# JohannesBuchner/massivedatans

Measured on AMD Instinct MI355X. Metric: likelihood evals/sec across N datasets per constrained draw, higher is better.
Workload: dtype f64

## Files before the change

### massivedatans_amd/csrc/mdns_chunk.hip

```cpp
#include "mdns_quad.h"
#include <cstdlib>

namespace mdns {

typedef JointMailbox ChunkMailbox;

template <int NST>
__global__ __launch_bounds__(256) void k_chunk_accept(
    const double *__restrict__ Y, int ld, int nx, int nxp, const double *__restrict__ xgrid,
    const double *__restrict__ params, int B, double scale,
    const int *__restrict__ rows, int *__restrict__ rows_dev, int M, int ntiles,
    const double *__restrict__ higher, int *__restrict__ flags, int stamp, JointTrail trail, JointHeader *__restrict__ header)
{
	extern __shared__ __attribute__((aligned(16))) double lds[];
	if (blockIdx.x == 0 && threadIdx.x == 0) header->status = 0;
	double2 *tpl = reinterpret_cast<double2 *>(lds);
	double *par = lds + (size_t) nxp * 4;
	unsigned long long *votes = reinterpret_cast<unsigned long long *>(par + 12);
	const int lane = threadIdx.x & 63, wave = threadIdx.x >> 6;
	const int q = lane & 3;
	const int bt = blockIdx.x / ntiles, tile = blockIdx.x - bt * ntiles;
	double pv = 0.0;
	if (threadIdx.x < 12) {
		const int b = bt * 4 + threadIdx.x / 3;
		pv = b < B ? params[(size_t) b * 3 + threadIdx.x % 3] : 0.0;
	}
	const int r = wave * 16 + (lane >> 2);
	const int k = tile * 64 + r;
	const bool live = k < M;
	const int kk = live ? k : M - 1;
	const int row = rows ? rows[kk] : kk;
	if (rows_dev && bt == 0 && live && q == 0) rows_dev[k] = row;
	double2 y[NST];
	const double thr = quad_load_row<NST>(Y, ld, row, live, q, higher, y);
	if (threadIdx.x < 12) par[threadIdx.x] = pv;
	__syncthreads();
	quad_templates(lds, par, xgrid, nx, nxp, bt * 4, B);
	__syncthreads();
	const double L = quad_sum<NST>(tpl, nxp / kCH, q, y) * scale;
	quad_vote(L, thr, bt * 4 + q < B, bt * 4 + q, true, bt * 4 + wave, ntiles, tile, r, votes, flags, stamp, trail);
}

__global__ __launch_bounds__(1024) void k_chunk_commit(
    const int *__restrict__ thr_rows, int M, int B, int ntiles, const int *__restrict__ flags, int stamp,
    JointTrail trail, JointArrays st, JointHeader *__restrict__ header, unsigned long long *__restrict__ fillbits,
    ChunkMailbox *__restrict__ box, unsigned long long seq)
{
	__shared__ int s_first, s_status;
	if (threadIdx.x == 0) s_status = 0;
	const int bstar = first_flagged<1024>(&s_first, flags, B, [=](int f) { return f == stamp; });
	const int lane = threadIdx.x & 63, wave = threadIdx.x >> 6;
	if (bstar < B) {
		for (int tile = wave; tile < ntiles; tile += 16) {
			const size_t at = (size_t) bstar * ntiles + tile;
			const unsigned long long word = trail.stamp_of[at] == trail.stamp ? trail.word[at] : 0ull;
			const int k = tile * 64 + lane;
			if (k < M && (word >> lane & 1ull)) {
				const int d = thr_rows ? thr_rows[k] : k;
				if (!shelf_append<16>(st, d, trail.L[at * 64 + lane], st.higher[d])) atomicOr(&s_status, 1);
			}
			if (lane == 0) { fillbits[tile] = word; mail_store(&box->bits[tile], word); }
		}
	}
	handover_release();
	__syncthreads();
	if (threadIdx.x != 0) return;
	const int accepted = bstar < B ? bstar : -1;
	header->accepted = accepted;
	header->status = s_status;
	mail_store(&box->accepted, accepted);
	mail_store(&box->status, s_status);
	mail_raise(&box->seq, seq);
}

typedef double double4_t __attribute__((ext_vector_type(4)));
typedef double double2_t __attribute__((ext_vector_type(2)));
__device__ __forceinline__ double4_t gg_join(double2_t a, double2_t b) { return double4_t{a[0], a[1], b[0], b[1]}; }

template <int SPEC, int CHUNK, int DEPTH, int PROBE>
__global__ __launch_bounds__(256) void k_gauss_mfma_filter(
    const double *__restrict__ YT, int nxp, int nx, const double *__restrict__ model_t, const double *__restrict__ msq, int B,
    double scale, const int *__restrict__ thr_rows, int M, int ntiles, int nbt, int ngroups,
    const double *__restrict__ higher, const double *__restrict__ ysq, int *__restrict__ flags, int *__restrict__ ambiguous,
    int stamp, int *__restrict__ lowest)
{
	constexpr int NB = SPEC / 16;
	constexpr int kRow2 = SPEC / 2;
	constexpr int kPieces = (CHUNK * kRow2 + 255) / 256;
	constexpr bool kWhole = (CHUNK * kRow2) % 256 == 0;
	constexpr int kRowsPerPass = 256 / kRow2;
	constexpr int kSteps = CHUNK / 4;
	__shared__ __attribute__((aligned(16))) double stage[DEPTH + 1][CHUNK * SPEC];
	const int lane = threadIdx.x & 63, wave = threadIdx.x >> 6;
	const int xcd = blockIdx.x & 7, local = blockIdx.x >> 3;
	const int tile = (local / ngroups) * 8 + xcd, grp = local - (local / ngroups) * ngroups;
	if (tile >= ntiles) return;
	const int bt = grp * 4 + wave;
	const bool working = bt < nbt;
	const int kq = lane >> 4, jq = lane & 15;
	const double *ap = model_t + (size_t) (working ? bt : 0) * nxp * 16 + lane;
	const int first = tile * SPEC;
	const int prow = threadIdx.x / kRow2, pcol = threadIdx.x % kRow2;
	const double2 *src = reinterpret_cast<const double2 *>(YT + ((size_t) (first >> 6) * nxp << 6) + (first & 63)) + (size_t) prow * 32 + pcol;
	double2 piece[DEPTH + 1][kPieces];
	double a[DEPTH + 1][kSteps];
	double4_t acc[NB];
#pragma unroll
	for (int t = 0; t < NB; t++) acc[t] = double4_t{0, 0, 0, 0};
	const int nchunks = (nxp + CHUNK - 1) / CHUNK;
	const int nk = nxp / 4;
#define FILTER_FETCH(SET, CHUNK_NO) { \
	const int cn_ = (CHUNK_NO) < nchunks ? (CHUNK_NO) : nchunks - 1; \
	_Pragma("unroll") for (int i = 0; i < kPieces; i++) { \
		const int row = kWhole || prow + i * kRowsPerPass < CHUNK ? prow + i * kRowsPerPass : CHUNK - 1; \
		const int ch = cn_ * CHUNK + row; \
		piece[SET][i] = src[(size_t) ((ch < nxp ? ch : nxp - 1) - prow) * 32]; \
	} \
	_Pragma("unroll") for (int i = 0; i < kSteps; i++) { \
		const int k = cn_ * kSteps + i; \
		a[SET][i] = ap[(size_t) (k < nk ? k : nk - 1) * 64]; \
	} }
#define FILTER_STAGE(SET, CHUNK_NO) { \
	const int cn_ = (CHUNK_NO) < nchunks ? (CHUNK_NO) : nchunks - 1; \
	_Pragma("unroll") for (int i = 0; i < kPieces; i++) { \
		const int row = prow + i * kRowsPerPass; \
		const bool inside = cn_ * CHUNK + row < nxp; \
		double2 v = piece[SET][i]; \
		v.x = inside ? v.x : 0.0; v.y = inside ? v.y : 0.0; \
		if (kWhole || row < CHUNK) reinterpret_cast<double2 *>(stage[SET])[i * 256 + threadIdx.x] = v; \
	} }
#define FILTER_BODY(R, R1, RF, CHUNK_NO) { \
	const int c_ = (CHUNK_NO); \
	if (PROBE != 2 && PROBE != 3) FILTER_FETCH(RF, c_ + DEPTH) \
	if (working && c_ < nchunks && PROBE != 1) { \
		const double *cur = stage[R]; \
		double b[2][NB]; \
		_Pragma("unroll") for (int t = 0; t < NB; t++) b[0][t] = cur[kq * SPEC + jq + 16 * t]; \
		_Pragma("unroll") for (int i = 0; i < kSteps; i++) { \
			if (i + 1 < kSteps) { \
				_Pragma("unroll") for (int t = 0; t < NB; t++) b[(i + 1) & 1][t] = cur[((i + 1) * 4 + kq) * SPEC + jq + 16 * t]; \
			} \
			 \
			_Pragma("unroll") for (int t = 0; t < NB; t++) \
				acc[t] = __builtin_amdgcn_mfma_f64_16x16x4f64(a[R][i], PROBE == 3 ? a[R][(i + t + 1) % kSteps] : b[i & 1][t], acc[t], 0, 0, 0); \
		} \
	} \
	if (PROBE != 2 && PROBE != 3) FILTER_STAGE(R1, c_ + 1) \
	__syncthreads(); }
	FILTER_FETCH(0, 0)
	if (DEPTH == 2) FILTER_FETCH(1, 1)
	FILTER_STAGE(0, 0)
	__syncthreads();
	if (DEPTH == 2) {
#pragma unroll 1
		for (int c = 0; c < nchunks; c += 3) {
			FILTER_BODY(0, 1, 2, c)
			FILTER_BODY(1, 2 % (DEPTH + 1), 0, c + 1)
			FILTER_BODY(2 % (DEPTH + 1), 0, 1, c + 2)
		}
	} else {
#pragma unroll 1
		for (int c = 0; c < nchunks; c += 2) {
			FILTER_BODY(0, 1, 1, c)
			FILTER_BODY(1, 0, 0, c + 1)
		}
	}
#undef FILTER_BODY
#undef FILTER_STAGE
#undef FILTER_FETCH
	if (!working) return;
	if (PROBE == 3) { double sum = 0.0; for (int t = 0; t < NB; t++) sum += acc[t][t]; if (sum == 12345.678) flags[0] = 1; return; }
	const double unit = fabs(scale) * (double) (nx + 8) * 0x1p-52;
	double mm[4];
#pragma unroll
	for (int v = 0; v < 4; v++) mm[v] = msq[bt * 16 + 4 * v + kq];
	bool hit[4] = {false, false, false, false}, maybe[4] = {false, false, false, false};
#pragma unroll
	for (int t = 0; t < NB; t++) {
		const int k = first + 16 * t + jq;
		const bool live = k < M;
		const int kk = live ? k : M - 1;
		const int d = thr_rows ? thr_rows[kk] : kk;
		const double thr = live ? higher[d] : __builtin_nan("");
		const double yy = ysq[d];
#pragma unroll
		for (int v = 0; v < 4; v++) {
			const double S = acc[t][v];
			const double Lf = scale * ((mm[v] - 2.0 * S) + yy);
			const double E4 = 4.0 * unit * ((mm[v] + 2.0 * fabs(S)) + yy);
			const bool valid = bt * 16 + 4 * v + kq < B;
			const bool h = valid && Lf > thr + E4;
			hit[v] = hit[v] || h;
			maybe[v] = maybe[v] || (valid && !h && Lf >= thr - E4);
		}
	}
	int best = 0x7fffffff;
#pragma unroll
	for (int v = 0; v < 4; v++) {
		const unsigned long long hm = __ballot(hit[v]), mb = __ballot(maybe[v]);
		if (lane == 0) {
#pragma unroll
			for (int g = 0; g < 4; g++) {
				const int cand = bt * 16 + 4 * v + g;
				if ((hm >> (16 * g)) & 0xffffull) { flags[cand] = 1; best = cand < best ? cand : best; }
				else if ((mb >> (16 * g)) & 0xffffull) ambiguous[cand] = stamp;
			}
		}
	}
	if (lane == 0 && best != 0x7fffffff) atomicMax(lowest, B - best);
}

template <int NC>
__global__ __launch_bounds__(256) void k_gauss_mfma_direct(
    const double *__restrict__ YT, int nxp, int nx, const double *__restrict__ model_t, const double *__restrict__ msq, int B,
    double scale, const int *__restrict__ thr_rows, int M, int nbt,
    const double *__restrict__ higher, const double *__restrict__ ysq, int *__restrict__ flags, int *__restrict__ ambiguous,
    int stamp, int *__restrict__ lowest, const double *__restrict__ zeros)
{
	const int lane = threadIdx.x & 63, wave = __builtin_amdgcn_readfirstlane((int) (threadIdx.x >> 6));
	const int i = lane & 15, q = lane >> 4;
	const int first = blockIdx.x * 16;
	const int ct0 = (blockIdx.y * 4 + wave) * NC;
	if (ct0 >= nbt) return;
	const int sp = first + i;
	const double *pa = YT + ((size_t) (sp >> 6) * nxp << 6) + (sp & 63);
	const double *pb[NC];
#pragma unroll
	for (int c = 0; c < NC; c++) pb[c] = model_t + (size_t) (ct0 + c < nbt ? ct0 + c : nbt - 1) * nxp * 16 + i;
	double4_t acc[NC];
#pragma unroll
	for (int c = 0; c < NC; c++) acc[c] = double4_t{0, 0, 0, 0};
	const int ng = (nxp + 15) >> 4;
	double a[2][4], b[2][NC][4];
#define GD_FETCH(SET, G) { \
	const int g_ = (G) < ng ? (G) : ng - 1; \
	_Pragma("unroll") for (int t = 0; t < 4; t++) { \
		const int ch = 16 * g_ + 4 * q + t; \
		const bool in = ch < nxp && (G) < ng; \
		a[SET][t] = *(in ? pa + ((size_t) ch << 6) : zeros + i); \
		const int cb = ch < nxp ? ch : nxp - 1; \
		_Pragma("unroll") for (int c = 0; c < NC; c++) b[SET][c][t] = pb[c][(size_t) cb << 4]; \
	} }
#define GD_BODY(SET) { \
	__builtin_amdgcn_sched_barrier(0); \
	_Pragma("unroll") for (int t = 0; t < 4; t++) \
		_Pragma("unroll") for (int c = 0; c < NC; c++) \
			acc[c] = __builtin_amdgcn_mfma_f64_16x16x4f64(a[SET][t], b[SET][c][t], acc[c], 0, 0, 0); \
	__builtin_amdgcn_sched_barrier(0); }
	GD_FETCH(0, 0)
#pragma unroll 1
	for (int g = 0; g < ng; g += 2) {
		GD_FETCH(1, g + 1)
		GD_BODY(0)
		GD_FETCH(0, g + 2)
		GD_BODY(1)
	}
#undef GD_BODY
#undef GD_FETCH
	const double unit = fabs(scale) * (double) (nx + 8) * 0x1p-52;
	double thr[4], yy[4];
#pragma unroll
	for (int v = 0; v < 4; v++) {
		const int k = first + 4 * v + q;
		const bool live = k < M;
		const int kk = live ? k : M - 1;
		const int d = thr_rows ? thr_rows[kk] : kk;
		thr[v] = live ? higher[d] : __builtin_nan("");
		yy[v] = ysq[d];
	}
	int best = 0x7fffffff;
#pragma unroll
	for (int c = 0; c < NC; c++) {
		const int cand = (ct0 + c) * 16 + i;
		const bool valid = ct0 + c < nbt && cand < B;
		const double mm = msq[valid ? cand : 0];
		bool hit = false, maybe = false;
#pragma unroll
		for (int v = 0; v < 4; v++) {
			const double S = acc[c][v];
			const double Lf = scale * ((mm - 2.0 * S) + yy[v]);
			const double E4 = 4.0 * unit * ((mm + 2.0 * fabs(S)) + yy[v]);
			const bool h = valid && Lf > thr[v] + E4;
			hit = hit || h;
			maybe = maybe || (valid && !h && Lf >= thr[v] - E4);
		}
		const unsigned long long hm = __ballot(hit), mb = __ballot(maybe);
		if (lane < 16) {
			const unsigned long long mine = 0x0001000100010001ull << lane;
			if (hm & mine) { flags[cand] = 1; best = cand < best ? cand : best; }
			else if (mb & mine) ambiguous[cand] = stamp;
		}
	}
#pragma unroll
	for (int off = 8; off > 0; off >>= 1) { const int o = __shfl_xor(best, off, 64); best = o < best ? o : best; }
	if (lane == 0 && best != 0x7fffffff) atomicMax(lowest, B - best);
}

template <int NC, bool KSPLIT>
__global__ __launch_bounds__(256) void k_gauss_gemm_filter(
    const double *__restrict__ YG, int nxg, int nx, const double *__restrict__ model_g, const double *__restrict__ msq, int B,
    double scale, const int *__restrict__ thr_rows, int M, int nbt,
    const double *__restrict__ higher, const double *__restrict__ ysq, int *__restrict__ flags, int *__restrict__ ambiguous,
    int stamp, int *__restrict__ lowest)
{
	__shared__ double red[KSPLIT ? 3 : 1][KSPLIT ? NC * 256 : 1];
	const int lane = threadIdx.x & 63, wave = __builtin_amdgcn_readfirstlane((int) (threadIdx.x >> 6));
	const int i = lane & 15, q = lane >> 4;
	const int rtile = KSPLIT ? blockIdx.x : blockIdx.x * 4 + wave;
	const int first = rtile * 16;
	if (first >= M) return;
	const int ct0 = blockIdx.y * NC;
	const int ncp = nxg >> 1, ng = nxg >> 4;
	const int g0 = KSPLIT ? (wave * ng) >> 2 : 0, g1 = KSPLIT ? ((wave + 1) * ng) >> 2 : ng;
	const double *pa = YG + (((size_t) rtile * ncp + 2 * q) << 5) + 2 * i;
	const double *pb[NC];
#pragma unroll
	for (int c = 0; c < NC; c++) pb[c] = model_g + (((size_t) (ct0 + c < nbt ? ct0 + c : nbt - 1) * ncp + 2 * q) << 5) + 2 * i;
	double4_t acc[NC];
#pragma unroll
	for (int c = 0; c < NC; c++) acc[c] = double4_t{0, 0, 0, 0};
	double4_t a[2], b[2][NC];
#define GG_LOAD4(P, G) gg_join(*reinterpret_cast<const double2_t *>((P) + ((size_t) (G) << 8)), *reinterpret_cast<const double2_t *>((P) + ((size_t) (G) << 8) + 32))
#define GG_FETCH(SET, G) { \
	const int g_ = (G) < g1 ? (G) : g1 - 1; \
	a[SET] = GG_LOAD4(pa, g_); \
	_Pragma("unroll") for (int c = 0; c < NC; c++) b[SET][c] = GG_LOAD4(pb[c], g_); }
#define GG_BODY(SET, G) { \
	__builtin_amdgcn_sched_barrier(0); \
	if ((G) < g1) { \
		_Pragma("unroll") for (int t = 0; t < 4; t++) \
			_Pragma("unroll") for (int c = 0; c < NC; c++) \
				acc[c] = __builtin_amdgcn_mfma_f64_16x16x4f64(a[SET][t], b[SET][c][t], acc[c], 0, 0, 0); \
	} \
	__builtin_amdgcn_sched_barrier(0); }
	if (g0 < g1) {
		GG_FETCH(0, g0)
#pragma unroll 1
		for (int g = g0; g < g1; g += 2) {
			GG_FETCH(1, g + 1)
			GG_BODY(0, g)
			GG_FETCH(0, g + 2)
			GG_BODY(1, g + 1)
		}
	}
#undef GG_BODY
#undef GG_FETCH
#undef GG_LOAD4
	if (KSPLIT) {
		if (wave != 0) {
#pragma unroll
			for (int c = 0; c < NC; c++)
#pragma unroll
				for (int v = 0; v < 4; v++) red[wave - 1][(c * 4 + v) * 64 + lane] = acc[c][v];
		}
		__syncthreads();
		if (wave != 0) return;
#pragma unroll
		for (int c = 0; c < NC; c++)
#pragma unroll
			for (int v = 0; v < 4; v++)
				acc[c][v] = ((acc[c][v] + red[0][(c * 4 + v) * 64 + lane]) + red[1][(c * 4 + v) * 64 + lane]) + red[2][(c * 4 + v) * 64 + lane];
	}
	const double unit = fabs(scale) * (double) (nx + 8) * 0x1p-52;
	double thr[4], yy[4];
#pragma unroll
	for (int v = 0; v < 4; v++) {
		const int k = first + 4 * v + q;
		const bool live = k < M;
		const int kk = live ? k : M - 1;
		const int d = thr_rows ? thr_rows[kk] : kk;
		thr[v] = live ? higher[d] : __builtin_nan("");
		yy[v] = ysq[d];
	}
	int best = 0x7fffffff;
#pragma unroll
	for (int c = 0; c < NC; c++) {
		const int cand = (ct0 + c) * 16 + i;
		const bool valid = ct0 + c < nbt && cand < B;
		const double mm = msq[valid ? cand : 0];
		bool hit = false, maybe = false;
#pragma unroll
		for (int v = 0; v < 4; v++) {
			const double S = acc[c][v];
			const double Lf = scale * ((mm - 2.0 * S) + yy[v]);
			const double E4 = 4.0 * unit * ((mm + 2.0 * fabs(S)) + yy[v]);
			const bool h = valid && Lf > thr[v] + E4;
			hit = hit || h;
			maybe = maybe || (valid && !h && Lf >= thr[v] - E4);
		}
		const unsigned long long hm = __ballot(hit), mb = __ballot(maybe);
		if (lane < 16) {
			const unsigned long long mine = 0x0001000100010001ull << lane;
			if (hm & mine) { flags[cand] = 1; best = cand < best ? cand : best; }
			else if (mb & mine) ambiguous[cand] = stamp;
		}
	}
#pragma unroll
	for (int off = 8; off > 0; off >>= 1) { const int o = __shfl_xor(best, off, 64); best = o < best ? o : best; }
	if (lane == 0 && best != 0x7fffffff) atomicMax(lowest, B - best);
}

static constexpr int kExactMost = 64;
template <int NST>
__global__ __launch_bounds__(256) void k_exact_list(
    const double *__restrict__ Y, int ld, int nxp, const double *__restrict__ model_t, double scale,
    const int *__restrict__ rows, int M, int ntiles, const double *__restrict__ higher, int B,
    const int *__restrict__ ambiguous, int stamp, const int *__restrict__ lowest, int *__restrict__ flags, JointTrail trail,
    JointHeader *__restrict__ header)
{
	extern __shared__ __attribute__((aligned(16))) double lds[];
	double2 *tpl = reinterpret_cast<double2 *>(lds);
	unsigned long long *votes = reinterpret_cast<unsigned long long *>(lds + (size_t) nxp * 4);
	__shared__ int list[kExactMost];
	__shared__ int s_n;
	const int lane = threadIdx.x & 63, wave = threadIdx.x >> 6;
	if (wave == 0) {
		const int low = *lowest > 0 ? B - *lowest : B;
		int n = 0;
		for (int b0 = 0; b0 < B && b0 <= low; b0 += 64) {
			const int b = b0 + lane;
			const bool take = b < B && ((b < low && ambiguous[b] == stamp) || b == low);
			const unsigned long long m = __ballot(take);
			if (take) {
				const int at = n + __popcll(m & ((1ull << lane) - 1ull));
				if (at < kExactMost) list[at] = b;
			}
			n += __popcll(m);
		}
		if (lane == 0) {
			s_n = n < kExactMost ? n : kExactMost;
			if (n > kExactMost && blockIdx.x == 0) atomicOr(&header->status, 2);
		}
	}
	__syncthreads();
	const int n = s_n;
	if (n == 0) return;
	const int q = lane & 3;
	const int tile = blockIdx.x;
	const int r = wave * 16 + (lane >> 2);
	const int k = tile * 64 + r;
	const bool live = k < M;
	const int kk = live ? k : M - 1;
	const int row = rows ? rows[kk] : kk;
	double2 y[NST];
	const double thr = quad_load_row<NST>(Y, ld, row, live, q, higher, y);
	for (int g = 0; g < n; g += 4) {
		quad_templates_listed(lds, model_t, nxp, list, g, n);
		__syncthreads();
		const double L = quad_sum<NST>(tpl, nxp / kCH, q, y) * scale;
		const bool has_q = g + q < n, has_w = g + wave < n;
		quad_vote(L, thr, has_q, has_q ? list[g + q] : -1, has_w, has_w ? list[g + wave] : -1, ntiles, tile, r, votes, flags, 1, trail);
		__syncthreads();
	}
}

bool chunk_fits(const mdns_spectra *s, int M, int B)
{
	Context *c = ctx();
	const int ntiles = (M + 63) / 64;
	const long long groups = (long long) ntiles * ((B + 3) / 4);
	static const char *limit = getenv("MDNS_CHUNK_GROUPS");
	const long long most = limit && atoll(limit) > 0 ? atoll(limit) : 16LL * c->num_cus;
	if (M > 4096 && B > 8) return false;
	return groups <= most && cols_nx(s->nx) <= 8 * 32 && s->d_x.get() != nullptr;
}

bool launch_chunk_accept(const mdns_spectra *s, const double *d_params_mapped, int B, double scale,
                         const int *d_rows_in, int *d_rows_dev, int M, const double *d_higher,
                         int *d_flags, int stamp, const JointTrail &trail, void *d_header)
{
	Context *c = ctx();
	const int ntiles = (M + 63) / 64;
	const int nbt = (B + 3) / 4;
	const int nxp = cols_nx(s->nx);
	const size_t lds = ((size_t) nxp * 4 + 12 + 4) * sizeof(double);
	const int nst = nxp / kCH;
	ProfileScope prof(0);
#define CHUNK_LAUNCH(NST) hipLaunchKernelGGL((k_chunk_accept<NST>), dim3(ntiles * nbt), dim3(256), lds, c->stream, \
	s->d_y.get(), s->ld, s->nx, nxp, s->d_x.get(), d_params_mapped, B, scale, d_rows_in, d_rows_dev, M, ntiles, d_higher, d_flags, stamp, trail, (JointHeader *) d_header)
	if (nst <= 8) { note_kernel(0, "k_chunk_accept<8>"); CHUNK_LAUNCH(8); }
	else if (nst <= 16) { note_kernel(0, "k_chunk_accept<16>"); CHUNK_LAUNCH(16); }
	else if (nst <= 26) { note_kernel(0, "k_chunk_accept<26>"); CHUNK_LAUNCH(26); }
	else { note_kernel(0, "k_chunk_accept<32>"); CHUNK_LAUNCH(32); }
#undef CHUNK_LAUNCH
	return launched("k_chunk_accept");
}

bool launch_chunk_commit(const int *d_thr_rows, int M, int B, const int *d_flags, int stamp, const JointTrail &trail,
                         const JointArrays &st, void *d_header, unsigned long long *d_fillbits, void *box_dev,
                         unsigned long long seq)
{
	Context *c = ctx();
	const int ntiles = (M + 63) / 64;
	hipLaunchKernelGGL(k_chunk_commit, dim3(1), dim3(1024), 0, c->stream, d_thr_rows, M, B, ntiles, d_flags, stamp, trail, st,
	                   (JointHeader *) d_header, d_fillbits, (ChunkMailbox *) box_dev, seq);
	return launched("k_chunk_commit");
}

int gauss_mfma_form()
{
	static int form = -1;
	if (form < 0) {
		const char *e = getenv("MDNS_K1_FILTER_FORM");
		form = e && e[0] == 'd' ? 1 : (e && e[0] == 'l' ? 0 : 2);
	}
	return form;
}

bool launch_gauss_mfma_filter(const mdns_spectra *s, const double *d_yT, const double *d_model_t, int B, double scale,
                              const int *d_thr_rows, int M, const double *d_higher, int *d_flags,
                              const double *d_msq, const JointTrail &trail, int *d_lowest, int *d_scratch, void *d_header,
                              const double *d_yG, const double *d_model_g)
{
	Context *c = ctx();
	const int ntiles = (M + 63) / 64, nbt = (B + 15) / 16;
	const int nxp = cols_nx(s->nx);
	int *d_amb = d_scratch;
	{
		static const char *probe = getenv("MDNS_FILTER_PROBE");
		const int pr = probe ? atoi(probe) : 0;
		if (pr == 0 && d_yG && d_model_g && gauss_mfma_form() == 2) {
			const int nxg = tiled16_nx(s->nx);
			static const char *ncf = getenv("MDNS_K1_GEMM_NC");
			int nc = nbt >= 2 ? 2 : 1;
			if (ncf && (atoi(ncf) == 1 || atoi(ncf) == 2 || atoi(ncf) == 4) && atoi(ncf) <= nbt) nc = atoi(ncf);
			ProfileScope prof(0);
			note_kernel(0, "k_gauss_gemm_filter<%d>", nc);
			static const char *ks = getenv("MDNS_K1_GEMM_KSPLIT");
			const bool ksplit = ks && ks[0] == '1';
			const int rt = (M + 15) / 16;
#define GG_LAUNCH(NC) do { if (ksplit) hipLaunchKernelGGL((k_gauss_gemm_filter<NC, true>), dim3(rt, (nbt + NC - 1) / NC), dim3(256), 0, c->stream, \
			d_yG, nxg, s->nx, d_model_g, d_msq, B, scale, d_thr_rows, M, nbt, d_higher, (const double *) s->d_ysq.get(), d_flags, d_amb, trail.stamp, d_lowest); \
		else hipLaunchKernelGGL((k_gauss_gemm_filter<NC, false>), dim3((rt + 3) / 4, (nbt + NC - 1) / NC), dim3(256), 0, c->stream, \
			d_yG, nxg, s->nx, d_model_g, d_msq, B, scale, d_thr_rows, M, nbt, d_higher, (const double *) s->d_ysq.get(), d_flags, d_amb, trail.stamp, d_lowest); } while (0)
			if (nc == 4) GG_LAUNCH(4); else if (nc == 2) GG_LAUNCH(2); else GG_LAUNCH(1);
#undef GG_LAUNCH
			if (!launched("k_gauss_gemm_filter")) return false;
		} else if (pr == 0 && gauss_mfma_form() == 1) {
			if (!c->mfma_zeros.fit_zeroed(16)) return false;
			const int nc = nbt >= 16 ? 4 : (nbt >= 8 ? 2 : 1);
			const int gy = (nbt + 4 * nc - 1) / (4 * nc);
			ProfileScope prof(0);
			note_kernel(0, "k_gauss_mfma_direct<%d>", nc);
#define GD_LAUNCH(NC) hipLaunchKernelGGL((k_gauss_mfma_direct<NC>), dim3((M + 15) / 16, gy), dim3(256), 0, c->stream, \
			d_yT, nxp, s->nx, d_model_t, d_msq, B, scale, d_thr_rows, M, nbt, d_higher, (const double *) s->d_ysq.get(), d_flags, d_amb, trail.stamp, d_lowest, \
			(const double *) c->mfma_zeros.get())
			if (nc == 4) GD_LAUNCH(4); else if (nc == 2) GD_LAUNCH(2); else GD_LAUNCH(1);
#undef GD_LAUNCH
			if (!launched("k_gauss_mfma_direct")) return false;
		} else {
		const int nspec = (M + 31) / 32;
		const int ngroups = (nbt + 3) / 4;
		const int blocks = 8 * ((nspec + 7) / 8) * ngroups;
		ProfileScope prof(0);
		note_kernel(0, "k_gauss_mfma_filter");
#define MFMA_LAUNCH(D, P) hipLaunchKernelGGL((k_gauss_mfma_filter<32, 32, D, P>), dim3(blocks), dim3(256), 0, c->stream, \
		                   d_yT, nxp, s->nx, d_model_t, d_msq, B, scale, d_thr_rows, M, nspec, nbt, ngroups, d_higher, \
		                   (const double *) s->d_ysq.get(), d_flags, d_amb, trail.stamp, d_lowest)
		const bool forty = pr == 0 && (nxp + 39) / 40 * 40 < (nxp + 31) / 32 * 32;
		if (forty) hipLaunchKernelGGL((k_gauss_mfma_filter<32, 40, 1, 0>), dim3(blocks), dim3(256), 0, c->stream,
		                              d_yT, nxp, s->nx, d_model_t, d_msq, B, scale, d_thr_rows, M, nspec, nbt, ngroups, d_higher,
		                              (const double *) s->d_ysq.get(), d_flags, d_amb, trail.stamp, d_lowest);
		else switch (pr) {
		case 1: MFMA_LAUNCH(1, 1); break;
		case 2: MFMA_LAUNCH(1, 2); break;
		case 3: MFMA_LAUNCH(1, 3); break;
		case 4: MFMA_LAUNCH(2, 0); break;
		case 5: MFMA_LAUNCH(1, 0); break;
		default: MFMA_LAUNCH(1, 0); break;
		}
#undef MFMA_LAUNCH
		if (!launched("k_gauss_mfma_filter")) return false;
		}
	}
	const size_t lds = ((size_t) nxp * 4 + 4) * sizeof(double);
	const int nst = nxp / kCH;
#define EXACT_LAUNCH(NST) hipLaunchKernelGGL((k_exact_list<NST>), dim3(ntiles), dim3(256), lds, c->stream, \
	s->d_y.get(), s->ld, nxp, d_model_t, scale, d_thr_rows, M, ntiles, d_higher, B, (const int *) d_amb, trail.stamp, (const int *) d_lowest, d_flags, trail, \
	(JointHeader *) d_header)
	if (nst <= 8) EXACT_LAUNCH(8); else if (nst <= 16) EXACT_LAUNCH(16); else if (nst <= 26) EXACT_LAUNCH(26); else EXACT_LAUNCH(32);
#undef EXACT_LAUNCH
	return launched("k_exact_list");
}

}
```

Baseline: 30.56 billion.

## Register-block GEMM filter over two row tiles with two-wave K split

Generalizes the MFMA GEMM filter kernel so each wave computes NS row tiles against NC candidate tiles, which reuses each loaded B fragment across two row tiles. By default, when nc==2 and M>16, pairs of waves also split the K dimension and reduce their partial sums through LDS. Loads are now issued at double2 granularity with a finer double-buffered pipeline, and a launch-bounds occupancy hint is added. In exchange it uses more accumulator registers, adds a __syncthreads-based reduction, and launches fewer blocks, which could lower parallelism when M is small.

```diff
diff --git a/massivedatans_amd/csrc/mdns_chunk.hip b/massivedatans_amd/csrc/mdns_chunk.hip
--- a/massivedatans_amd/csrc/mdns_chunk.hip
+++ b/massivedatans_amd/csrc/mdns_chunk.hip
@@ -296,99 +296,124 @@
 	if (lane == 0 && best != 0x7fffffff) atomicMax(lowest, B - best);
 }
 
-template <int NC, bool KSPLIT>
-__global__ __launch_bounds__(256) void k_gauss_gemm_filter(
+template <int NS, int NC, int KW>
+__global__ __launch_bounds__(256, NS == 2 ? 5 : 1) void k_gauss_gemm_filter(
     const double *__restrict__ YG, int nxg, int nx, const double *__restrict__ model_g, const double *__restrict__ msq, int B,
     double scale, const int *__restrict__ thr_rows, int M, int nbt,
     const double *__restrict__ higher, const double *__restrict__ ysq, int *__restrict__ flags, int *__restrict__ ambiguous,
     int stamp, int *__restrict__ lowest)
 {
-	__shared__ double red[KSPLIT ? 3 : 1][KSPLIT ? NC * 256 : 1];
+	constexpr int kBlocks = 4 / KW;
+	constexpr int kAcc = NS * NC * 4;
+	__shared__ double red[KW > 1 ? kBlocks * (KW - 1) : 1][KW > 1 ? kAcc * 64 : 1];
 	const int lane = threadIdx.x & 63, wave = __builtin_amdgcn_readfirstlane((int) (threadIdx.x >> 6));
 	const int i = lane & 15, q = lane >> 4;
-	const int rtile = KSPLIT ? blockIdx.x : blockIdx.x * 4 + wave;
+	const int blk = wave / KW, part = wave % KW;
+	const int rt = (M + 15) >> 4;
+	const int rtile = (blockIdx.x * kBlocks + blk) * NS;
 	const int first = rtile * 16;
-	if (first >= M) return;
+	const bool active = first < M;
+	if (KW == 1 && !active) return;
 	const int ct0 = blockIdx.y * NC;
 	const int ncp = nxg >> 1, ng = nxg >> 4;
-	const int g0 = KSPLIT ? (wave * ng) >> 2 : 0, g1 = KSPLIT ? ((wave + 1) * ng) >> 2 : ng;
-	const double *pa = YG + (((size_t) rtile * ncp + 2 * q) << 5) + 2 * i;
-	const double *pb[NC];
+	const int g0 = KW > 1 ? (part * ng) / KW : 0, g1 = !active ? g0 : (KW > 1 ? ((part + 1) * ng) / KW : ng);
+	const double *pa[NS], *pb[NC];
+#pragma unroll
+	for (int s = 0; s < NS; s++) pa[s] = YG + (((size_t) (rtile + s < rt ? rtile + s : rt - 1) * ncp + 2 * q) << 5) + 2 * i;
 #pragma unroll
 	for (int c = 0; c < NC; c++) pb[c] = model_g + (((size_t) (ct0 + c < nbt ? ct0 + c : nbt - 1) * ncp + 2 * q) << 5) + 2 * i;
-	double4_t acc[NC];
-#pragma unroll
-	for (int c = 0; c < NC; c++) acc[c] = double4_t{0, 0, 0, 0};
-	double4_t a[2], b[2][NC];
-#define GG_LOAD4(P, G) gg_join(*reinterpret_cast<const double2_t *>((P) + ((size_t) (G) << 8)), *reinterpret_cast<const double2_t *>((P) + ((size_t) (G) << 8) + 32))
-#define GG_FETCH(SET, G) { \
+	double4_t acc[NS][NC];
+#pragma unroll
+	for (int s = 0; s < NS; s++)
+#pragma unroll
+		for (int c = 0; c < NC; c++) acc[s][c] = double4_t{0, 0, 0, 0};
+	double2_t a[2][NS], b[2][NC];
+#define GG_FETCH(SET, G, H) { \
 	const int g_ = (G) < g1 ? (G) : g1 - 1; \
-	a[SET] = GG_LOAD4(pa, g_); \
-	_Pragma("unroll") for (int c = 0; c < NC; c++) b[SET][c] = GG_LOAD4(pb[c], g_); }
-#define GG_BODY(SET, G) { \
+	_Pragma("unroll") for (int s = 0; s < NS; s++) a[SET][s] = *reinterpret_cast<const double2_t *>(pa[s] + ((size_t) g_ << 8) + 32 * (H)); \
+	_Pragma("unroll") for (int c = 0; c < NC; c++) b[SET][c] = *reinterpret_cast<const double2_t *>(pb[c] + ((size_t) g_ << 8) + 32 * (H)); }
+#define GG_BODY(SET) { \
 	__builtin_amdgcn_sched_barrier(0); \
-	if ((G) < g1) { \
-		_Pragma("unroll") for (int t = 0; t < 4; t++) \
+	_Pragma("unroll") for (int t = 0; t < 2; t++) \
+		_Pragma("unroll") for (int s = 0; s < NS; s++) \
 			_Pragma("unroll") for (int c = 0; c < NC; c++) \
-				acc[c] = __builtin_amdgcn_mfma_f64_16x16x4f64(a[SET][t], b[SET][c][t], acc[c], 0, 0, 0); \
-	} \
+				acc[s][c] = __builtin_amdgcn_mfma_f64_16x16x4f64(a[SET][s][t], b[SET][c][t], acc[s][c], 0, 0, 0); \
 	__builtin_amdgcn_sched_barrier(0); }
 	if (g0 < g1) {
-		GG_FETCH(0, g0)
+		GG_FETCH(0, g0, 0)
 #pragma unroll 1
-		for (int g = g0; g < g1; g += 2) {
-			GG_FETCH(1, g + 1)
-			GG_BODY(0, g)
-			GG_FETCH(0, g + 2)
-			GG_BODY(1, g + 1)
+		for (int g = g0; g < g1; g++) {
+			GG_FETCH(1, g, 1)
+			GG_BODY(0)
+			GG_FETCH(0, g + 1, 0)
+			GG_BODY(1)
 		}
 	}
 #undef GG_BODY
 #undef GG_FETCH
-#undef GG_LOAD4
-	if (KSPLIT) {
-		if (wave != 0) {
+	bool valid[NC];
+	double mm[NC], thr[NS][4], yy[NS][4];
+	if (part == 0 && active) {
+#pragma unroll
+		for (int c = 0; c < NC; c++) {
+			valid[c] = ct0 + c < nbt && (ct0 + c) * 16 + i < B;
+			mm[c] = msq[valid[c] ? (ct0 + c) * 16 + i : 0];
+		}
+#pragma unroll
+		for (int s = 0; s < NS; s++)
+#pragma unroll
+			for (int v = 0; v < 4; v++) {
+				const int k = first + 16 * s + 4 * v + q;
+				const bool live = k < M;
+				const int kk = live ? k : M - 1;
+				const int d = thr_rows ? thr_rows[kk] : kk;
+				thr[s][v] = live ? higher[d] : __builtin_nan("");
+				yy[s][v] = ysq[d];
+			}
+	}
+	if (KW > 1) {
+		if (part != 0 && active) {
+#pragma unroll
+			for (int s = 0; s < NS; s++)
+#pragma unroll
+				for (int c = 0; c < NC; c++)
+#pragma unroll
+					for (int v = 0; v < 4; v++) red[blk * (KW - 1) + part - 1][((s * NC + c) * 4 + v) * 64 + lane] = acc[s][c][v];
+		}
+		__syncthreads();
+	}
+	if (part != 0 || !active) return;
+	const double unit = fabs(scale) * (double) (nx + 8) * 0x1p-52;
+	bool hit[NC], maybe[NC];
+#pragma unroll
+	for (int c = 0; c < NC; c++) hit[c] = maybe[c] = false;
+#pragma unroll
+	for (int s = 0; s < NS; s++) {
+		if (KW > 1) {
 #pragma unroll
 			for (int c = 0; c < NC; c++)
 #pragma unroll
-				for (int v = 0; v < 4; v++) red[wave - 1][(c * 4 + v) * 64 + lane] = acc[c][v];
-		}
-		__syncthreads();
-		if (wave != 0) return;
+				for (int v = 0; v < 4; v++)
+#pragma unroll
+					for (int w = 0; w < KW - 1; w++) acc[s][c][v] += red[blk * (KW - 1) + w][((s * NC + c) * 4 + v) * 64 + lane];
+		}
 #pragma unroll
 		for (int c = 0; c < NC; c++)
 #pragma unroll
-			for (int v = 0; v < 4; v++)
-				acc[c][v] = ((acc[c][v] + red[0][(c * 4 + v) * 64 + lane]) + red[1][(c * 4 + v) * 64 + lane]) + red[2][(c * 4 + v) * 64 + lane];
-	}
-	const double unit = fabs(scale) * (double) (nx + 8) * 0x1p-52;
-	double thr[4], yy[4];
-#pragma unroll
-	for (int v = 0; v < 4; v++) {
-		const int k = first + 4 * v + q;
-		const bool live = k < M;
-		const int kk = live ? k : M - 1;
-		const int d = thr_rows ? thr_rows[kk] : kk;
-		thr[v] = live ? higher[d] : __builtin_nan("");
-		yy[v] = ysq[d];
+			for (int v = 0; v < 4; v++) {
+				const double S = acc[s][c][v];
+				const double Lf = scale * ((mm[c] - 2.0 * S) + yy[s][v]);
+				const double E4 = 4.0 * unit * ((mm[c] + 2.0 * fabs(S)) + yy[s][v]);
+				const bool h = valid[c] && Lf > thr[s][v] + E4;
+				hit[c] = hit[c] || h;
+				maybe[c] = maybe[c] || (valid[c] && !h && Lf >= thr[s][v] - E4);
+			}
 	}
 	int best = 0x7fffffff;
 #pragma unroll
 	for (int c = 0; c < NC; c++) {
 		const int cand = (ct0 + c) * 16 + i;
-		const bool valid = ct0 + c < nbt && cand < B;
-		const double mm = msq[valid ? cand : 0];
-		bool hit = false, maybe = false;
-#pragma unroll
-		for (int v = 0; v < 4; v++) {
-			const double S = acc[c][v];
-			const double Lf = scale * ((mm - 2.0 * S) + yy[v]);
-			const double E4 = 4.0 * unit * ((mm + 2.0 * fabs(S)) + yy[v]);
-			const bool h = valid && Lf > thr[v] + E4;
-			hit = hit || h;
-			maybe = maybe || (valid && !h && Lf >= thr[v] - E4);
-		}
-		const unsigned long long hm = __ballot(hit), mb = __ballot(maybe);
+		const unsigned long long hm = __ballot(hit[c]), mb = __ballot(maybe[c]);
 		if (lane < 16) {
 			const unsigned long long mine = 0x0001000100010001ull << lane;
 			if (hm & mine) { flags[cand] = 1; best = cand < best ? cand : best; }
@@ -524,16 +549,17 @@
 			static const char *ncf = getenv("MDNS_K1_GEMM_NC");
 			int nc = nbt >= 2 ? 2 : 1;
 			if (ncf && (atoi(ncf) == 1 || atoi(ncf) == 2 || atoi(ncf) == 4) && atoi(ncf) <= nbt) nc = atoi(ncf);
-			ProfileScope prof(0);
-			note_kernel(0, "k_gauss_gemm_filter<%d>", nc);
 			static const char *ks = getenv("MDNS_K1_GEMM_KSPLIT");
 			const bool ksplit = ks && ks[0] == '1';
+			const bool blocked = !ksplit && nc == 2 && M > 16;
+			ProfileScope prof(0);
+			note_kernel(0, "k_gauss_gemm_filter<%d,%d,%d>", blocked ? 2 : 1, nc, blocked ? 2 : (ksplit ? 4 : 1));
 			const int rt = (M + 15) / 16;
-#define GG_LAUNCH(NC) do { if (ksplit) hipLaunchKernelGGL((k_gauss_gemm_filter<NC, true>), dim3(rt, (nbt + NC - 1) / NC), dim3(256), 0, c->stream, \
-			d_yG, nxg, s->nx, d_model_g, d_msq, B, scale, d_thr_rows, M, nbt, d_higher, (const double *) s->d_ysq.get(), d_flags, d_amb, trail.stamp, d_lowest); \
-		else hipLaunchKernelGGL((k_gauss_gemm_filter<NC, false>), dim3((rt + 3) / 4, (nbt + NC - 1) / NC), dim3(256), 0, c->stream, \
-			d_yG, nxg, s->nx, d_model_g, d_msq, B, scale, d_thr_rows, M, nbt, d_higher, (const double *) s->d_ysq.get(), d_flags, d_amb, trail.stamp, d_lowest); } while (0)
-			if (nc == 4) GG_LAUNCH(4); else if (nc == 2) GG_LAUNCH(2); else GG_LAUNCH(1);
+#define GG_LAUNCH(NS, NC, KW) hipLaunchKernelGGL((k_gauss_gemm_filter<NS, NC, KW>), dim3((rt + NS * (4 / KW) - 1) / (NS * (4 / KW)), (nbt + NC - 1) / NC), dim3(256), 0, c->stream, \
+			d_yG, nxg, s->nx, d_model_g, d_msq, B, scale, d_thr_rows, M, nbt, d_higher, (const double *) s->d_ysq.get(), d_flags, d_amb, trail.stamp, d_lowest)
+#define GG_FORMS(NC) do { if (ksplit) GG_LAUNCH(1, NC, 4); else GG_LAUNCH(1, NC, 1); } while (0)
+			if (blocked) GG_LAUNCH(2, 2, 2); else if (nc == 4) GG_FORMS(4); else if (nc == 2) GG_FORMS(2); else GG_FORMS(1);
+#undef GG_FORMS
 #undef GG_LAUNCH
 			if (!launched("k_gauss_gemm_filter")) return false;
 		} else if (pr == 0 && gauss_mfma_form() == 1) {
```

Measured after the change: 30.48 billion. Within noise of the previous version (-0.3%).
